# timsainb/noisereduce

Hardware: AMD Instinct MI355X
Metric: Msamples/s reduce_noise (48 kHz mono, n_fft=1024) (higher is better)
Workload: dtype f32

## Files before the change

noisereduce_amd/csrc/api.hip:

```cpp
#include <hip/hip_runtime.h>
#include <dlfcn.h>

#include <algorithm>
#include <cmath>
#include <cstdarg>
#include <cstdio>
#include <cstring>
#include <map>
#include <mutex>
#include <string>
#include <vector>

#include "../../include/mi355gate_debug.h"
#pragma clang fp contract(on)
#include "kernels.hpp"
#include "fused.hpp"
#include "czt.hpp"
#include "mixed.hpp"
#include "onepass.hpp"
#include "rowgate.hpp"
#include "rowbwd.hpp"
#include "fast512.hpp"
#include "onepass512.hpp"
#include "fast256.hpp"
// ... 2147 lines not shown
  P.inv_ktot = 1.0f / (float)h->ktot;
#if OP_WHO
  if (!g_who_dev) HIPCHK(h, hipMalloc((void**)&g_who_dev, 4096 * 16));
  HIPCHK(h, hipMemsetAsync(g_who_dev, 0, 4096 * 16, st));
  P.who = g_who_dev;
#endif
#if OP_TRACE
  {
    static unsigned* tr = nullptr;
    static size_t tr_slots = 0;
    const size_t slots = (size_t)ub * ntt * 4;
    if (!tr || tr_slots < slots) {
      HIPCHK(h, hipMalloc((void**)&tr, slots * 64));
      tr_slots = slots;
      static unsigned** trp = &tr;
      static size_t* trn = &tr_slots;
      static bool reg = false;
      if (!reg) {
        reg = true;
        atexit([] {
          std::vector<unsigned> hst(*trn * 16);
          if (hipMemcpy(hst.data(), *trp, hst.size() * 4, hipMemcpyDeviceToHost) != hipSuccess) return;
          double sum[14] = {0}, w = 0, mx = 0;
          for (size_t i = 0; i < *trn; ++i) {
            if (hst[i * 16 + 15] != 1u) continue;
            w += 1;
            double tot = 0;
            for (int k = 0; k < 14; ++k) { sum[k] += hst[i * 16 + k]; tot += hst[i * 16 + k]; }
            mx = std::max(mx, tot);
          }
          fprintf(stderr, "[OP_TRACE] completed waves %.0f; average shader cycles per wave and phase:", w);
          double tot = 0;
          for (int k = 0; k < 14; ++k) { fprintf(stderr, " %d:%.0f", k, sum[k] / (w > 0 ? w : 1)); tot += sum[k] / (w > 0 ? w : 1); }
          fprintf(stderr, "  sum %.0f  longest wave %.0f\n", tot, mx);
        });
      }
    }
    HIPCHK(h, hipMemsetAsync(tr, 0, slots * 64, st));
    P.trace = tr;
    g_trace_dev = tr; g_trace_tiles = (size_t)ub * ntt; g_trace_ntt = (int)ntt;
  }
#endif
  {
    ProfScope ps(h, SG_STAGE_ONEPASS, st);
    const size_t lds = (size_t)(fast::FN + WAVES * fast::WAVE_CX_H) * sizeof(fast::cf) + (1024 + T2_FLOATS) * sizeof(float) +
                       256 * 8 + 514 * 8 + 32 + (prop ? 528 : 0);
    auto go = [&](auto kern) -> hipError_t {
      hipError_t e = set_lds(reinterpret_cast<const void*>(kern), lds);
      if (e != hipSuccess) return e;
      hipLaunchKernelGGL(kern, dim3(persist ? pgrid : (unsigned)(ub * ntt)), dim3(WAVES * 64), lds, st, P);
      return hipGetLastError();
    };
    if (persist && prop) HIPCHK(h, go(fast::k_gate_onepass<WAVES, true, false, false, true>));
    else if (persist) HIPCHK(h, go(fast::k_gate_onepass<WAVES, false, false, false, true>));
    else if (h->lose_now & 3u) HIPCHK(h, go(fast::k_gate_onepass<WAVES, false, true>));
    else if (prop) HIPCHK(h, go(fast::k_gate_onepass<WAVES, true>));
    else HIPCHK(h, go(fast::k_gate_onepass<WAVES, false>));
  }
  if (lazy) {
    ProfScope ps(h, SG_STAGE_STFT_MAX, st);
    const int wpr = (g.F + 63) / 64;
    HIPCHK(h, launch_bits_any<0>(h, vx, g, ub, tc,
                             (unsigned long long*)h->pmax.p, (unsigned long long*)h->bits.p, wpr, st));
    if ((rc = handoff_next_epoch(h, st))) return rc;
    P.epoch = h->epoch;
    P.ticket = (unsigned*)h->xticket.p + 8;
    P.ticket_base = 0;
    const size_t lds = (size_t)(fast::FN + WAVES * fast::WAVE_CX_H) * sizeof(fast::cf) + (1024 + T2_FLOATS) * sizeof(float) +
                       256 * 8 + 514 * 8 + 32 + (prop ? 528 : 0);
    auto redo = [&](auto kern) -> hipError_t {
      hipError_t e = set_lds(reinterpret_cast<const void*>(kern), lds);
      if (e != hipSuccess) return e;
      hipLaunchKernelGGL(kern, dim3((unsigned)(ub * ntt)), dim3(WAVES * 64), lds, st, P);
      return hipGetLastError();
    };
    if (prop) HIPCHK(h, redo(fast::k_gate_onepass<WAVES, true, false, true>));
    else HIPCHK(h, redo(fast::k_gate_onepass<WAVES, false, false, true>));
    HIPCHK(h, hipGetLastError());
  }
  h->dbg_xbits = true;
  h->dbg_trows = 16; h->dbg_tstep = 16; h->dbg_twords = fast::OP_TILE_WORDS; h->dbg_txw = fast::OP_XW;
  h->dbg_tf0 = A.h_begin - 3;
  h->dbg_ntt = (int)ntt;
  h->dbg_db = std::max<int64_t>(0, A.h_begin - 3 - NF);
  h->dbg_de = std::min<int64_t>(g.T, A.h_begin - 3 + NF * (n_tiles + 1));
  return SG_OK;
}

template <int WAVES, bool KMASK>
static hipError_t launch_apply_fast64(fast::Apply64Args& A, int64_t nh, int64_t ub, hipStream_t st) {
  constexpr int NH = 4 * WAVES - 3;
  const size_t lds = (size_t)(fast::FN + WAVES * 4 * fast::FSLOTS_D + 17) * sizeof(fast::cd);
// ... 1328 lines not shown
```

noisereduce_amd/csrc/onepass.hpp:

```cpp
#pragma once
#include "fastpath.hpp"

namespace sg {
namespace fast {

constexpr int OP_XW = 9;
constexpr int OP_TILE_WORDS = 16 * OP_XW * 2;
constexpr int OP_MAX_NT = 16;
constexpr int OP_KP = 528;
constexpr int OP_TAB_WIN = 0, OP_TAB_WSQ = 4096, OP_TAB_INVN = 8192, OP_TAB_TW512 = 9216, OP_TAB_TW1024 = 13312,
              OP_TAB_WIN64 = 17408, OP_TAB_TW64 = 25600, OP_TAB_MCONST = 33792, OP_TAB_EXP8 = 35328, OP_TAB_BYTES = 37376;

#ifndef OP_LATE_ARGS
#define OP_LATE_ARGS 1
#endif
#ifndef OP_TRACE
#define OP_TRACE 0
#endif
#ifndef OP_ARGCHECK
#define OP_ARGCHECK 0
#endif
#ifndef OP_TILECOUNT
#define OP_TILECOUNT 0
#endif
#ifndef OP_NO_LOOPTOP_WAIT
#define OP_NO_LOOPTOP_WAIT 0
#endif
#ifndef OP_BACKOFF
#define OP_BACKOFF 0
#endif
#if OP_BACKOFF
#define OP_POLL_SLEEP(spin) do { if ((spin) >= 8) __builtin_amdgcn_s_sleep(127); else __builtin_amdgcn_s_sleep(1); } while (0)
#else
#define OP_POLL_SLEEP(spin) __builtin_amdgcn_s_sleep(1)
#endif
#ifndef OP_WHO
#define OP_WHO 0
#endif
#ifndef OP_GLOBAL_DRAW
#define OP_GLOBAL_DRAW 0
#endif
#if OP_GLOBAL_DRAW
#define OP_DRAW_TICKET(p64) __hip_atomic_fetch_add((__attribute__((address_space(1))) unsigned*)(p64), 1u, __ATOMIC_RELAXED, __HIP_MEMORY_SCOPE_AGENT)
#else
#define OP_DRAW_TICKET(p64) atomicAdd((unsigned*)(uintptr_t)(p64), 1u)
#endif
#ifndef OP_DRAW_TOP
#define OP_DRAW_TOP 0
#endif
#ifndef OP_RESTAGE
#define OP_RESTAGE 0
#endif
#ifndef OP_MAX_ITERS
#define OP_MAX_ITERS 0
#endif
#ifndef OP_LATE_START_US
#define OP_LATE_START_US 0
#endif
#ifndef OP_EXP_STALL_NS
#define OP_EXP_STALL_NS 0
#endif
#ifndef OP_INPLACE
#define OP_INPLACE 0
#endif
struct OnePassArgs {
  ApplyArgs A;
  const void* x_exact;
  int64_t stride_exact;
// ... 30 lines not shown
#if OP_LATE_ARGS
  const __attribute__((address_space(4))) char* kp4 = (const __attribute__((address_space(4))) char*)__builtin_amdgcn_kernarg_segment_ptr();
  asm volatile("" : "+s"(kp4));
#endif
  const int64_t s0 = t * OP_XARG(int32_t, A.g.H) - OP_XARG(int32_t, A.g.padL);
  const int64_t v_cs = OP_XARG(int64_t, A.view.cs), v_pad = OP_XARG(int64_t, A.view.pad), v_Lp = OP_XARG(int64_t, A.view.Lp),
                v_lo = OP_XARG(int64_t, A.view.lo), v_hi = OP_XARG(int64_t, A.view.hi), x_stride = OP_XARG(int64_t, stride_exact);
  const void* const x_exact = (const void*)(uintptr_t)OP_XARG(unsigned long long, x_exact);
  const int x_dtype = OP_XARG(int, dtype_exact);
  const char* const tab = (const char*)(uintptr_t)OP_XARG(unsigned long long, tab);
  const int64_t e = chunk * v_cs - v_pad + s0;
  int a, b;
  exact1024_terms(s0, e, v_Lp, v_lo, v_hi, a, b);
  return exact1024_power(x_exact, x_dtype, row * x_stride + e, a, b, reinterpret_cast<const double*>(tab + OP_TAB_WIN64),
                         reinterpret_cast<const cx<double>*>(tab + OP_TAB_TW64), f, lane);
}

__device__ __forceinline__ unsigned op_nan_bits() {
  unsigned v = 0x7fc00000u;
  asm volatile("" : "+v"(v));
  return v;
}

#ifndef OP_ABLATE
#define OP_ABLATE 0
#endif
#ifndef OP_TRACE
#define OP_TRACE 0
#endif
#if OP_TRACE
#define OP_STAMP(i)                                                                                   \
  do {                                                                                                \
    const long long t_now_ = clock64();                                                               \
    if (lane == 0 && t_slot_) t_slot_[i] = (unsigned)(t_now_ - t_prev_);                              \
    t_prev_ = t_now_;                                                                                 \
  } while (0)
#else
#define OP_STAMP(i) do { } while (0)
#endif

#ifndef OP_LATE_P
#define OP_LATE_P 1
#endif
#ifndef OP_OCC
#define OP_OCC 3
#endif
#define OP_DONE { if (PERSIST) continue; return; }
#ifndef OP_DEFER_SEAM
#define OP_DEFER_SEAM 1
#endif
constexpr unsigned OP_SEAM_NONE = 0xffffffffu;
template <int WAVES, bool PROP, bool LOSE = false, bool REDO = false, bool PERSIST = false>
__global__ __launch_bounds__(WAVES * 64, OP_OCC) void k_gate_onepass(OnePassArgs Pk) {
  static_assert(WAVES == 4, "tile = 16 frames");
  static_assert(!PERSIST || (!LOSE && !REDO), "the persistent loop is the lazy first launch only");
  extern __shared__ __attribute__((aligned(16))) char smem[];
  cf* tw512 = reinterpret_cast<cf*>(smem);
  cf* regions = tw512 + FN;
  float* swin = reinterpret_cast<float*>(regions + WAVES * WAVE_CX_H);
  float* s_t2 = swin + 1024;
  unsigned long long* s_exp = reinterpret_cast<unsigned long long*>(s_t2 + T2_FLOATS);
  double* s_t2d = reinterpret_cast<double*>(s_exp + 256);
  unsigned* s_misc = reinterpret_cast<unsigned*>(s_t2d + 514);
  unsigned char* s_ef = reinterpret_cast<unsigned char*>(s_misc + 8);
  constexpr int NF = 4 * WAVES;
  constexpr int SPAN = (NF - 1) * 256 + 1024, XPITCH = 288;
  static_assert((SPAN / 256) * XPITCH <= WAVES * WAVE_CX_H * 2, "span must fit the exchange slices");
  constexpr int NQ = SPAN / 256;
  static_assert(SPAN % 256 == 0 && WAVES * 64 == 256, "one sample per thread and row");
  constexpr int SCAN_REG = 5;

  if (REDO && Pk.alim[1] != Pk.tc.need_tag) return;
#if OP_LATE_START_US
  if (PERSIST && (blockIdx.x % 5u) == 1u) {
    const unsigned long long t0_ = wall_clock64();
    while ((long long)(wall_clock64() - t0_) < (long long)OP_LATE_START_US * 100 * (1 + (blockIdx.x % 7u))) __builtin_amdgcn_s_sleep(8);
  }
#endif
  double t2pre[3];
  unsigned alim_v = 0u;
  {
    const int tid = threadIdx.x, lane = tid & 63;
    static_assert(FN == 2 * WAVES * 64 && WAVES * 64 == 256, "one pass of the prologue loads per thread");
    const cf tw_a = reinterpret_cast<const cf*>(Pk.tab + OP_TAB_TW512)[(tid >> 4) * (tid & 15)];
    const cf tw_b = reinterpret_cast<const cf*>(Pk.tab + OP_TAB_TW512)[((tid + 256) >> 4) * (tid & 15)];
    const float4 w4 = reinterpret_cast<const float4*>(Pk.tab + OP_TAB_WIN)[tid];
    const unsigned long long e8 = reinterpret_cast<const unsigned long long*>(Pk.tab + OP_TAB_EXP8)[tid];
    t2pre[0] = Pk.tc.T2[perm_inv(tid)];
    t2pre[1] = Pk.tc.T2[perm_inv(tid + 256)];
    t2pre[2] = Pk.tc.T2[perm_inv(512)];
    if (!REDO && Pk.alim != nullptr) {
      int z = 2 + min(lane & 15, OP_ALIM_BLOCKS - 1);
      asm volatile("" : "+v"(z));
      alim_v = Pk.alim[z];
    }
    if (tid == 0) {
      s_misc[PERSIST ? 4 : 0] = Pk.ticket_base == 0xffffffffu ? blockIdx.x : atomicAdd(Pk.ticket, 1u) - Pk.ticket_base;
      s_misc[1] = 0u;
      if (PERSIST) s_misc[0] = OP_SEAM_NONE;
    }
    tw512[tid] = tw_a;
    tw512[tid + 256] = tw_b;
    reinterpret_cast<float4*>(swin)[tid] = w4;
    s_exp[tid] = e8;
    if constexpr (PROP) {
      for (int f = tid; f <= 512; f += WAVES * 64) {
        const int lo = max(-Pk.nf, -f), hi = min(Pk.nf, 512 - f);
        int sum = 0;
        for (int a = lo; a <= hi; ++a) sum += Pk.nf + 1 - (a < 0 ? -a : a);
        s_ef[f] = (unsigned char)sum;
      }
    }
    if constexpr (PERSIST) {
#pragma unroll
      for (int k = 0; k < 3; ++k) {
        const int i = tid + k * WAVES * 64;
        if (i > 512) break;
        s_t2[t2_pos(i)] = t2_to_f32(t2pre[k], 4.0);
        s_t2d[i] = t2pre[k];
      }
      for (int off = 1; off < 16; off <<= 1) alim_v = min(alim_v, (unsigned)__shfl_xor((int)alim_v, off));
      if (tid == 0) s_misc[2] = alim_v;
#if OP_TILECOUNT == 2
      if (tid == 0) { s_misc[3] = Pk.total_tiles; s_misc[6] = (unsigned)(uintptr_t)Pk.err; s_misc[7] = (unsigned)((uintptr_t)Pk.err >> 32); }
#endif
    }
  }
// ... 65 lines not shown
                      (rowq * OP_QARG(int64_t, A.om.stride) + gi00 - OP_QARG(int64_t, A.om.g0)));
    src = (const unsigned long long*)uni((const unsigned long long*)(uintptr_t)OP_QARG(unsigned long long, part2) +
                                         ((size_t)uq * ntl + jq - 1) * 3 * 256);
  };
  auto seam_off = [](int wv, int s4_) -> int { return wv * 256 + s4_; };
  auto seam_finish = [&](unsigned pend, int wv, int s4_, unsigned long long g0_, unsigned long long g1_, unsigned long long g2_,
                        unsigned long long g3_, float* dst, float4 ld, float4 nrm) {
    op_v4u ga = {(unsigned)g0_, (unsigned)(g0_ >> 32), (unsigned)g1_, (unsigned)(g1_ >> 32)};
    op_v4u gb = {(unsigned)g2_, (unsigned)(g2_ >> 32), (unsigned)g3_, (unsigned)(g3_ >> 32)};
    typedef const __attribute__((address_space(4))) char* kq_t;
    kq_t kq = (kq_t)__builtin_amdgcn_kernarg_segment_ptr();
    asm volatile("" : "+s"(kq));
    const unsigned e = OP_QARG(unsigned, epoch);
    if (!(ga[1] == e && ga[3] == e && gb[1] == e && gb[3] == e)) {
      const unsigned long long* src;
      float* d2_;
      seam_where(pend, src, d2_);
      src += seam_off(wv, s4_);
      for (int spin = 0;; ++spin) {
        asm volatile("global_load_dwordx4 %0, %2, off sc1\n\tglobal_load_dwordx4 %1, %2, off offset:16 sc1\n\ts_waitcnt vmcnt(0)"
                     : "=&v"(ga), "=&v"(gb) : "v"(src) : "memory");
        if (ga[1] == e && ga[3] == e && gb[1] == e && gb[3] == e) break;
        if (spin >= OP_SPIN_MAX) {
          atomicOr_system((unsigned*)(uintptr_t)OP_QARG(unsigned long long, err), 2u);
          ga[0] = ga[2] = gb[0] = gb[2] = op_nan_bits();
          break;
        }
        OP_POLL_SLEEP(spin);
      }
    }
    const float psn = __uint_as_float((pend >> 31) * 0x7fc00000u);
    float4 a;
    a.x = __uint_as_float(ga[0]) + ld.x;
    a.y = __uint_as_float(ga[2]) + ld.y;
    a.z = __uint_as_float(gb[0]) + ld.z;
    a.w = __uint_as_float(gb[2]) + ld.w;
    a.x = (a.x + psn) * nrm.x; a.y = (a.y + psn) * nrm.y; a.z = (a.z + psn) * nrm.z; a.w = (a.w + psn) * nrm.w;
    *reinterpret_cast<float4*>(dst + seam_off(wv, s4_)) = a;
  };
  auto seam_close = [&](unsigned pend, int tid_) {
    const int wv = tid_ >> 6, s4_ = (tid_ & 63) * 4;
    if (pend == OP_SEAM_NONE || wv >= 3) return;
    typedef const __attribute__((address_space(4))) char* kq_t;
    kq_t kq = (kq_t)__builtin_amdgcn_kernarg_segment_ptr();
    asm volatile("" : "+s"(kq));
    const float4 nrm = *reinterpret_cast<const float4*>(
        &reinterpret_cast<const float*>((const char*)(uintptr_t)OP_QARG(unsigned long long, tab) + OP_TAB_INVN)[s4_]);
    const unsigned long long* src;
    float* dst;
    seam_where(pend, src, dst);
    const float4 ld = *reinterpret_cast<const float4*>(dst + seam_off(wv, s4_));
    seam_finish(pend, wv, s4_, 0ull, 0ull, 0ull, 0ull, dst, ld, nrm);
  };

#if OP_EXP_STALL_NS
  const unsigned long long op_exp_t0_ = wall_clock64();
#endif
  for (unsigned iter = 0; iter == 0u || PERSIST; ++iter) {
  const OnePassArgs& P = (PERSIST || OP_LATE_P) ? *late_args<OnePassArgs>() : Pk;
  int tid = threadIdx.x;
#if OP_ARGCHECK
#if OP_ARGCHECK == 2
  if (PERSIST && threadIdx.x == 1) {
    const unsigned* a_ = reinterpret_cast<const unsigned*>(&P);
    const unsigned* b_ = reinterpret_cast<const unsigned*>(&Pk);
    bool same_ = true;
    for (unsigned w_ = 0; w_ < sizeof(OnePassArgs) / 4; ++w_) same_ = same_ && a_[w_] == b_[w_];
    if (!same_) atomicOr_system(Pk.err, 0x80u);
  }
#else
  if (PERSIST && threadIdx.x == 0 && (P.total_tiles != Pk.total_tiles || P.epoch != Pk.epoch || P.xbits != Pk.xbits || P.A.view.x != Pk.A.view.x))
    atomicOr_system(Pk.err, 0x80u);
#endif
#endif
// ... 29 lines not shown
    atomicOr_system(e_, 0x40u);
    atomicMax_system(e_ + 6, P.total_tiles);
    atomicMax_system(e_ + 7, iter);
  }
  if (PERSIST && ticket >= s_misc[3]) return;
#endif
#if OP_WHO
  if (PERSIST && threadIdx.x == 0 && ticket < 4096u) P.who[ticket * 4 + 2] = (blockIdx.x + 1u) | (iter << 16);
#endif
  if (PERSIST && ticket >= P.total_tiles) {
    if constexpr (DEFER) seam_close((unsigned)__builtin_amdgcn_readfirstlane((int)s_misc[0]), tid);
    return;
  }
#if OP_TILECOUNT == 1
  if (PERSIST && threadIdx.x == 0) { atomicAdd_system(P.err + 4, 1u); atomicAdd_system(P.err + 5, ticket); }
#endif
#if OP_RESTAGE
  if (PERSIST && iter != 0u) {
    const int t_ = threadIdx.x;
    tw512[t_] = reinterpret_cast<const cf*>(P.tab + OP_TAB_TW512)[(t_ >> 4) * (t_ & 15)];
    tw512[t_ + 256] = reinterpret_cast<const cf*>(P.tab + OP_TAB_TW512)[((t_ + 256) >> 4) * (t_ & 15)];
    reinterpret_cast<float4*>(swin)[t_] = reinterpret_cast<const float4*>(P.tab + OP_TAB_WIN)[t_];
    s_exp[t_] = reinterpret_cast<const unsigned long long*>(P.tab + OP_TAB_EXP8)[t_];
#pragma unroll
    for (int k = 0; k < 3; ++k) {
      const int i = t_ + k * WAVES * 64;
      if (i > 512) break;
      const double v_ = P.tc.T2[perm_inv(i)];
      s_t2[t2_pos(i)] = t2_to_f32(v_, 4.0);
      s_t2d[i] = v_;
    }
  }
#endif
  if (PERSIST && tid == 0) {
    s_misc[1] = 0u;
#if OP_TK_LATE
    s_misc[tk_slot ^ 1u] = 0xffffffffu;
#endif
  }
#if OP_TRACE
  t_slot_ = P.trace + ((size_t)ticket * 4 + wave) * 16;
  if (lane == 0) t_slot_[14] = (blockIdx.x + 1u) | (iter << 16);
#endif
  OP_STAMP(0);
  const int64_t u = ticket / (unsigned)ntt;
  const int jt = (int)(ticket % (unsigned)ntt) - 1;
// ... 100 lines not shown
    const float2* wl = reinterpret_cast<const float2*>(swin + 2 * c);
    if (blk_vec) {
#pragma unroll
      for (int r = 0; r < 32; ++r) {
        const float2 x2 = *reinterpret_cast<const float2*>(xs + (r >> 3) * XPITCH + 32 * (r & 7));
        const float2 w2 = wl[16 * r];
        v[r] = {x2.x * w2.x, x2.y * w2.y};
      }
    } else {
#pragma unroll
      for (int r = 0; r < 32; ++r) {
        float2 x2 = *reinterpret_cast<const float2*>(xs + (r >> 3) * XPITCH + 32 * (r & 7));
        if (!fvalid) x2 = make_float2(0.f, 0.f);
        const float2 w2 = wl[16 * r];
        v[r] = {x2.x * w2.x, x2.y * w2.y};
      }
    }
  }
  __syncthreads();
  OP_STAMP(2);
  {
#pragma unroll
    for (int r = 0; r < 32; ++r) nrm2 += v[r].x * v[r].x + v[r].y * v[r].y;
    nrm2 += __shfl_xor(nrm2, 1);
    nrm2 += __shfl_xor(nrm2, 2);
    nrm2 += __shfl_xor(nrm2, 4);
    nrm2 += __shfl_xor(nrm2, 8);
  }
  {
    int z0 = 0;
    asm volatile("" : "+v"(z0));
    fft512_fwd_half(v, fb, tw512 + z0, c);
  }
  OP_STAMP(3);

#if OP_INPLACE
  const bool l0 = c == 0;
  cf wlo = reinterpret_cast<const cf*>(P.tab + OP_TAB_TW1024)[c];
  asm volatile("" : "+v"(wlo.x), "+v"(wlo.y));
  cf whi = wlo;
  {
    const cf w16 = reinterpret_cast<const cf*>(P.tab + OP_TAB_TW1024)[16];
    if (l0) whi = {-w16.y, w16.x};
  }
  rg_lane0_to_entries(v, l0);
  {
    const cf r0 = v[0], r31 = v[31];
    cf xa, xb;
    split_pair(r0, r31, wlo, xa, xb);
    v[0] = {l0 ? r0.x : xa.x, l0 ? r0.y : xa.y};
// ... 104 lines not shown
        const double Pe = op_exact_power(P, row, chunk, tq + gs, f, lane);
        const bool pass = Pe > s_t2d[q < 32 ? cs * 32 + q : 512];
        if (lane == src) {
          if (q < 32) {
            pred = (pred & ~(1u << q)) | ((pass ? 1u : 0u) << q);
            amb &= ~(1u << q);
          } else {
            pred512 = pass;
            amb512 = false;
          }
        }
      }
      wave_lds_sync();
#pragma unroll
      for (int i = 0; i < 16; ++i) {
        OP_PB(i).x = park[(2 * i) * 64];
        OP_PB(i).y = park[(2 * i + 1) * 64];
      }
      wave_lds_sync();
    }
    if (l0)
      pred = (pred & 0xffu) | ((pred & 0x00ffff00u) << 8) | ((pred >> 15) & 0xfe00u) | ((pred >> 23) & 0x100u);
    unsigned tr = pred;
    auto tstep = [&](int sft, unsigned msk, unsigned long long up) {
      const unsigned y = (unsigned)__shfl_xor((int)tr, sft);
      const unsigned ysh = sel_s(up, y >> sft, y << sft);
      const unsigned mk = sel_s(up, msk, ~msk);
      tr = (tr & ~mk) | (ysh & mk);
    };
    tstep(8, 0x00ff00ffu, 0xff00ff00ff00ff00ull);
    tstep(4, 0x0f0f0f0fu, 0xf0f0f0f0f0f0f0f0ull);
    tstep(2, 0x33333333u, 0xccccccccccccccccull);
    tstep(1, 0x55555555u, 0xaaaaaaaaaaaaaaaaull);
    const unsigned long long b8 = __ballot(pred512);
    {
      const int sh = 16 * g;
      const int srcl = (lane & 48) | ((2 * c) & 15);
      const unsigned wa = (unsigned)__shfl((int)tr, srcl), wb2 = (unsigned)__shfl((int)tr, srcl + 1);
      const unsigned f0 = wa & 0xffffu, f1 = wa >> 16, f2 = wb2 & 0xffffu, f3 = wb2 >> 16;
      const unsigned r1 = (((__brev(f1) >> 16) << 1) | (f1 & 1u)) & 0xffffu;
      const unsigned r3 = (((__brev(f3) >> 16) << 1) | (f3 & 1u)) & 0xffffu;
      myword = (unsigned long long)(f0 | (r1 << 16)) | ((unsigned long long)(f2 | (r3 << 16)) << 32);
      if (c == 8) myword = (b8 >> sh) & 1ull;
    }
  }

  OP_STAMP(5);
#if OP_LATE_ARGS
  typedef const __attribute__((address_space(4))) char* op_kpm_t;
  op_kpm_t kpm = (op_kpm_t)__builtin_amdgcn_kernarg_segment_ptr();
  asm volatile("" : "+s"(kpm));
#define OP_MARG(type, member) (*(const __attribute__((address_space(4))) type*)(kpm + __builtin_offsetof(OnePassArgs, member)))
  const unsigned m_ticket = (unsigned)__builtin_amdgcn_readfirstlane((int)s_misc[tk_slot]);
  const unsigned m_ntt = (unsigned)(OP_MARG(int, A.n_tiles) + 2);
  const int64_t m_u = m_ticket / m_ntt;
  const int m_jt = (int)(m_ticket % m_ntt) - 1;
// ... 9 lines not shown
  const char* const m_tab = (const char*)(uintptr_t)OP_MARG(unsigned long long, tab);
  const float m_kscale = OP_MARG(float, A.kscale);
  const int m_nt = OP_MARG(int, nt);
  [[maybe_unused]] const float m_inv_ktot = OP_MARG(float, inv_ktot), m_prop = OP_MARG(float, prop);
  unsigned long long* xb_mine = m_xbits + ((size_t)m_u * m_ntt + (m_jt + 1)) * OP_TILE_WORDS;
  if (c < OP_XW) {
    const op_v4u gr = {(unsigned)myword, m_epoch, (unsigned)(myword >> 32), m_epoch};
    op_st16_sc1(&xb_mine[((4 * wave + g) * OP_XW + c) * 2], gr);
  }
  [[maybe_unused]] unsigned pend_halo = OP_SEAM_NONE;
  if constexpr (DEFER) {
    if (halo_tile) pend_halo = (unsigned)__builtin_amdgcn_readfirstlane((int)s_misc[0]);
  }
  __syncthreads();
  if (halo_tile) {
    if constexpr (DEFER) {
      seam_close(pend_halo, tid);
      if (tid == 0) s_misc[0] = OP_SEAM_NONE;
    }
    if constexpr (PERSIST) {
#if OP_MAX_ITERS == 1 || OP_DRAW_TOP
      if (tid == 0) s_misc[tk_slot ^ 1u] = 0xffffffffu;
#else
      if (tid == 0) s_misc[tk_slot ^ 1u] = OP_DRAW_TICKET(OP_MARG(unsigned long long, ticket)) - OP_MARG(unsigned, ticket_base);
#endif
      pf = false;
#pragma unroll
      for (int k = 0; k < NQ; ++k) q[k] = 0.f;
#pragma unroll
      for (int k = 0; k < SCAN_REG; ++k) sc[k] = 0.f;
    }
    OP_DONE;
  }
  OP_STAMP(6);

  constexpr int WP = OP_XW + 2;
  constexpr int WPB = WP * 8;
  constexpr int SLICE_B = WAVE_CX_H * 8;
  char* rbytes = reinterpret_cast<char*>(regions);
  unsigned long long* wb = reinterpret_cast<unsigned long long*>(rbytes + 4 * OP_KP * 2);
  static_assert(4 * OP_KP * 2 + 48 * WPB <= SLICE_B, "bit rows must fit behind wave 0's K rows");
  const unsigned char* wbb = reinterpret_cast<const unsigned char*>(wb);
  if (c < OP_XW) wb[(m_nt + 4 * wave + g) * WP + 1 + c] = myword;
  for (int r = tid; r < 48; r += WAVES * 64) {
    wb[r * WP] = 0ull;
    wb[r * WP + WP - 1] = 0ull;
  }
  const int q4 = lane >> 4, j16 = lane & 15;
  const long Bf = (long)reinterpret_cast<const unsigned long long*>(m_tab + OP_TAB_MCONST)[lane], At1 = (long)reinterpret_cast<const unsigned long long*>(m_tab + OP_TAB_MCONST)[64 + lane], At2 = (long)reinterpret_cast<const unsigned long long*>(m_tab + OP_TAB_MCONST)[128 + lane];
  const bool three = 2 * m_nt > 16;
  const int m1 = j16, m2 = 16 + j16;
  const int r1 = m1 < 2 * m_nt ? (m1 < m_nt ? m1 : 16 + m1) : 0;
  const int r2 = m2 < 2 * m_nt ? (m2 < m_nt ? m2 : 16 + m2) : 0;
  __syncthreads();
  typedef int op_v4i __attribute__((ext_vector_type(4)));
  const op_v4i zero4 = {0, 0, 0, 0};
  unsigned hown[9];
  {
    const unsigned char* rp = wbb + (m_nt + j16) * WPB + 7 + q4;
#pragma unroll
    for (int nb = 0; nb < 9; ++nb) {
      const int b = wave + 4 * nb;
      hown[nb] = 0u;
      if (b < 33) {
        const long a = (long)s_exp[rp[2 * b]];
        const op_v4i h = __builtin_amdgcn_mfma_i32_16x16x32_i8(a, Bf, zero4, 0, 0, 0);
        hown[nb] = (unsigned)h[0] | ((unsigned)h[1] << 8) | ((unsigned)h[2] << 16) | ((unsigned)h[3] << 24);
      }
    }
  }
  OP_STAMP(7);
  for (int i = tid; i < 2 * m_nt * OP_XW; i += WAVES * 64) {
    const int side = i >= m_nt * OP_XW;
    const int rem = i - side * m_nt * OP_XW;
    const int rr = rem / OP_XW, w = rem - rr * OP_XW;
    const unsigned long long* src = side ? xb_mine + OP_TILE_WORDS + (rr * OP_XW + w) * 2
                                         : xb_mine - OP_TILE_WORDS + ((NF - m_nt + rr) * OP_XW + w) * 2;
    op_v4u gr = op_ld16_sc1(src);
    for (int spin = 0; !(OP_ABLATE & 2) && (LOSE || gr[1] != m_epoch || gr[3] != m_epoch); ++spin) {
      if (LOSE || spin >= OP_SPIN_MAX) {
        atomicOr_system(m_err, 1u);
#if OP_WHO
        if (atomicAdd_system(m_err + 14, 1u) == 0u) { m_err[8] = m_ticket; m_err[9] = (unsigned)i; m_err[10] = gr[1]; m_err[11] = m_epoch; }
#endif
        s_misc[1] = 1u;
        break;
      }
      OP_POLL_SLEEP(spin);
      gr = op_ld16_sc1(src);
    }
    wb[(side ? m_nt + NF + rr : rr) * WP + 1 + w] = (unsigned long long)gr[0] | ((unsigned long long)gr[2] << 32);
  }
  __syncthreads();
  OP_STAMP(8);
  [[maybe_unused]] unsigned nx_raw = 0u;
  if constexpr (PERSIST) {
#if OP_MAX_ITERS == 1 || OP_DRAW_TOP
    if (tid == 0) nx_raw = 0xffffffffu + OP_MARG(unsigned, ticket_base);
#else
    if (tid == 0) nx_raw = OP_DRAW_TICKET(OP_MARG(unsigned long long, ticket));
#endif
  }
  {
    const unsigned char* rp1 = wbb + r1 * WPB + 7 + q4;
    const unsigned char* rp2 = wbb + r2 * WPB + 7 + q4;
#pragma unroll
    for (int nb = 0; nb < 9; ++nb) {
      const int b = wave + 4 * nb;
      if (b < 33) {
        const long a1 = (long)s_exp[rp1[2 * b]];
        const op_v4i h1 = __builtin_amdgcn_mfma_i32_16x16x32_i8(a1, Bf, zero4, 0, 0, 0);
        const unsigned p1 = (unsigned)h1[0] | ((unsigned)h1[1] << 8) | ((unsigned)h1[2] << 16) | ((unsigned)h1[3] << 24);
        const long bt1 = (long)(((unsigned long long)p1 << 32) | (unsigned long long)hown[nb]);
        op_v4i d = __builtin_amdgcn_mfma_i32_16x16x32_i8(At1, bt1, zero4, 0, 0, 0);
        if (three) {
          const long a2 = (long)s_exp[rp2[2 * b]];
          const op_v4i h2 = __builtin_amdgcn_mfma_i32_16x16x32_i8(a2, Bf, zero4, 0, 0, 0);
          const unsigned p2 = (unsigned)h2[0] | ((unsigned)h2[1] << 8) | ((unsigned)h2[2] << 16) | ((unsigned)h2[3] << 24);
          d = __builtin_amdgcn_mfma_i32_16x16x32_i8(At2, (long)(unsigned long long)p2, d, 0, 0, 0);
        }
        unsigned short* kd = reinterpret_cast<unsigned short*>(rbytes + q4 * (SLICE_B + 64)) + 16 * b + j16;
        kd[0] = (unsigned short)d[0];
        kd[OP_KP] = (unsigned short)d[1];
// ... 92 lines not shown
    for (int i = 9; i < 16; ++i) v[i] = sel(pb[16 - i], pa[i]);
#pragma unroll
    for (int i = 16; i < 24; ++i) v[i] = sel(pa[i - 8], pb[31 - i]);
#pragma unroll
    for (int i = 24; i < 31; ++i) v[i] = sel(pb[39 - i], pb[31 - i]);
    v[31] = sel(pb[8], pb[0]);
  }
#endif
  wave_lds_sync();
  OP_STAMP(10);
#if OP_TK_LATE
  if constexpr (PERSIST) {
    if (tid == 0) *(volatile unsigned*)&s_misc[tk_slot ^ 1u] = nx_raw - OP_MARG(unsigned, ticket_base);
  }
#endif

  {
    int zi = 0, ci = c;
    asm volatile("" : "+v"(zi), "+v"(ci));
    fft512_inv_half(v, fb + zi, tw512 + zi, ci);
  }
  OP_STAMP(11);
  float4 n4;
  auto load_n4 = [&]() { n4 = *reinterpret_cast<const float4*>(&reinterpret_cast<const float*>(m_tab + OP_TAB_INVN)[(tid & 63) * 4]); };
  if constexpr (PERSIST) load_n4();
  auto prefetch_next = [&]() {
    const OnePassArgs& Pn = *late_args<OnePassArgs>();
#if OP_TK_LATE
    unsigned nx_v;
    while ((nx_v = *(volatile unsigned*)&s_misc[tk_slot ^ 1u]) == 0xffffffffu) __builtin_amdgcn_s_sleep(1);
    const unsigned nx = (unsigned)__builtin_amdgcn_readfirstlane((int)nx_v);
#else
    const unsigned nx = (unsigned)__builtin_amdgcn_readfirstlane((int)s_misc[tk_slot ^ 1u]);
#endif
    pf = true;
    const bool n_live = nx < Pn.total_tiles;
    const unsigned n_ntt = (unsigned)(Pn.A.n_tiles + 2);
    const unsigned n_tk = n_live ? nx : 0u;
    const unsigned n_u = n_tk / n_ntt;
    const int n_jt = (int)(n_tk % n_ntt) - 1;
    const unsigned n_gu = (unsigned)(Pn.A.view.unit0 + n_u), n_nch = (unsigned)Pn.A.view.n_chunks;
    const TileSrc N = tile_src(Pn, (int64_t)(n_gu / n_nch), Pn.A.view.c0 + n_gu % n_nch, n_jt, true);
    if (n_live && N.blk_vec) {
#pragma unroll
      for (int k = 0; k < NQ; ++k) q[k] = N.sp[tid + k * 256];
    } else {
#pragma unroll
      for (int k = 0; k < NQ; ++k) q[k] = 0.f;
    }
    if (n_live && N.sc_base != nullptr) {
#pragma unroll
      for (int k = 0; k < SCAN_REG; ++k) sc[k] = N.sc_base[min(tid + k * WAVES * 64, N.sc_n1)];
    } else {
#pragma unroll
      for (int k = 0; k < SCAN_REG; ++k) sc[k] = 0.f;
    }
  };
#ifndef OP_PF_AT
#define OP_PF_AT 2
#endif
#ifndef OP_TK_LATE
#define OP_TK_LATE 0
#endif
#ifndef OP_SEAM_AT
#define OP_SEAM_AT 4
#endif
  [[maybe_unused]] unsigned sm_pend = OP_SEAM_NONE;
  [[maybe_unused]] unsigned long long sm_g0 = 0ull, sm_g1 = 0ull, sm_g2 = 0ull, sm_g3 = 0ull;
  [[maybe_unused]] float* sm_dst = nullptr;
  [[maybe_unused]] float4 sm_lead = make_float4(0.f, 0.f, 0.f, 0.f);
  auto seam_issue = [&]() {
    sm_pend = (unsigned)__builtin_amdgcn_readfirstlane((int)s_misc[0]);
    if (sm_pend != OP_SEAM_NONE && wave < 3) {
      const unsigned long long* sm_src;
      seam_where(sm_pend, sm_src, sm_dst);
      sm_src += seam_off(wave, (tid & 63) * 4);
      sm_g0 = __hip_atomic_load((const __attribute__((address_space(1))) unsigned long long*)(sm_src), __ATOMIC_RELAXED, __HIP_MEMORY_SCOPE_AGENT);
      sm_g1 = __hip_atomic_load((const __attribute__((address_space(1))) unsigned long long*)(sm_src + 1), __ATOMIC_RELAXED, __HIP_MEMORY_SCOPE_AGENT);
      sm_g2 = __hip_atomic_load((const __attribute__((address_space(1))) unsigned long long*)(sm_src + 2), __ATOMIC_RELAXED, __HIP_MEMORY_SCOPE_AGENT);
      sm_g3 = __hip_atomic_load((const __attribute__((address_space(1))) unsigned long long*)(sm_src + 3), __ATOMIC_RELAXED, __HIP_MEMORY_SCOPE_AGENT);
      typedef float op_v4f __attribute__((ext_vector_type(4)));
      const op_v4f l4 = *(const __attribute__((address_space(1))) op_v4f*)(sm_dst + seam_off(wave, (tid & 63) * 4));
      sm_lead = make_float4(l4[0], l4[1], l4[2], l4[3]);
    }
  };
  if constexpr (PERSIST && OP_PF_AT == 0) prefetch_next();
  float* acc = reinterpret_cast<float*>(regions + wave * WAVE_CX_H);
  {
    const float2* wsrc2 = reinterpret_cast<const float2*>(swin + 2 * c);
#pragma unroll
    for (int j = 0; j < 4; ++j) {
#pragma unroll
      for (int rr = 0; rr < 8; ++rr) {
        const int r = 8 * j + rr;
        float2* dst = reinterpret_cast<float2*>(acc + (g + j) * HPITCH + 2 * c + 32 * rr);
        const float2 ws = wsrc2[16 * r];
        float2 nw = {v[r].x * ws.x, v[r].y * ws.y};
        if (j != 0) {
          const float2 old = *dst;
          nw.x = sel_s(OLA_KEEP, nw.x + old.x, nw.x);
          nw.y = sel_s(OLA_KEEP, nw.y + old.y, nw.y);
        }
        *dst = nw;
      }
      wave_lds_sync();
      if constexpr (PERSIST) { if (j + 1 == OP_PF_AT) prefetch_next(); }
// ... 42 lines not shown
  const int64_t e_u = u, e_row = row, e_chunk = chunk, e_tf = tf_tile;
  const int e_jt = jt;
  [[maybe_unused]] const unsigned e_ticket = ticket;
#endif
  const float* fr = reinterpret_cast<const float*>(regions);
  const int s4 = (tid & 63) * 4;
  unsigned poison_u = __builtin_amdgcn_readfirstlane((int)s_misc[1]) != 0 ? 0x7fc00000u : 0u;
  asm volatile("" : "+s"(poison_u));
  const float poison = __uint_as_float(poison_u);
  {
    const int64_t pb0 = e_tf * 256 - e_padL;
    const int64_t gi00 = e_chunk * e_gstep + (pb0 - e_p0);
    float* dbase = (float*)e_out + (e_row * e_ostride + gi00 - e_g0);
    float* dst0 = dbase + s4;
    const bool tile_fast = e_odtype == 0 && e_normalize && e_tf >= 3 && e_tf + NF + 2 < e_T &&
                           e_tf >= e_hbegin && e_tf + NF + 2 < e_hend && pb0 >= e_p0 &&
                           pb0 + NF * 256 <= e_p1 && pb0 + NF * 256 <= e_Lout && gi00 >= e_glo &&
                           gi00 + NF * 256 <= e_ghi && (reinterpret_cast<uintptr_t>(dbase) & 15) == 0 && WAVES == 4;
    if (tile_fast) {
      constexpr int R = WAVE_CX_H * 2;
      auto ld4 = [&](int off) { return *reinterpret_cast<const float4*>(&fr[off + s4]); };
      auto fin = [&](float4 a, int jj) {
        a.x = (a.x + poison) * n4.x; a.y = (a.y + poison) * n4.y; a.z = (a.z + poison) * n4.z; a.w = (a.w + poison) * n4.w;
        *reinterpret_cast<float4*>(dst0 + jj * 256) = a;
      };
      if (wave == 3) {
#pragma unroll
        for (int it = 0; it < 4; ++it) fin(ld4(it * R + 3 * HPITCH), 3 + 4 * it);
        OP_STAMP(13);
        if constexpr (PERSIST && OP_PF_AT == 5) prefetch_next();
        OP_DONE;
      }
      {
        const float4 a4 = ld4((WAVES - 1) * R + (wave + 4) * HPITCH);
        unsigned long long* dst = e_part2 + (((size_t)e_u * e_ntiles + e_jt) * 3 + wave) * 256 + s4;
        const op_v4u ga = {__float_as_uint(a4.x + poison), e_epoch, __float_as_uint(a4.y + poison), e_epoch};
        const op_v4u gb = {__float_as_uint(a4.z + poison), e_epoch, __float_as_uint(a4.w + poison), e_epoch};
        op_st16_sc1(dst, ga);
        op_st16_sc1(dst + 2, gb);
      }
#pragma unroll
      for (int it = 1; it < 4; ++it) {
        float4 a4 = ld4((it - 1) * R + (wave + 4) * HPITCH);
        const float4 f4 = ld4(it * R + wave * HPITCH);
        a4.x += f4.x; a4.y += f4.y; a4.z += f4.z; a4.w += f4.w;
        fin(a4, wave + 4 * it);
      }
      if constexpr (DEFER) {
        if (sm_pend != OP_SEAM_NONE) seam_finish(sm_pend, wave, s4, sm_g0, sm_g1, sm_g2, sm_g3, sm_dst, sm_lead, n4);
        *reinterpret_cast<float4*>(dst0 + wave * 256) = ld4(wave * HPITCH);
        if (tid == 0) s_misc[0] = e_ticket | (s_misc[1] != 0u ? 0x80000000u : 0u);
      } else {
        float4 a4 = ld4(wave * HPITCH);
        const unsigned long long* src = e_part2 + (((size_t)e_u * e_ntiles + e_jt - 1) * 3 + wave) * 256 + s4;
        op_v4u ga, gb;
        for (int spin = 0;; ++spin) {
          asm volatile("global_load_dwordx4 %0, %2, off sc1\n\tglobal_load_dwordx4 %1, %2, off offset:16 sc1\n\ts_waitcnt vmcnt(0)"
                       : "=&v"(ga), "=&v"(gb) : "v"(src) : "memory");
          const unsigned e = e_epoch;
          if ((OP_ABLATE & 16) || (!LOSE && ga[1] == e && ga[3] == e && gb[1] == e && gb[3] == e)) break;
          if (LOSE || spin >= OP_SPIN_MAX) {
            atomicOr_system(e_err, 2u);
#if OP_WHO
            if (atomicAdd_system(e_err + 15, 1u) == 0u) { e_err[12] = e_ticket; e_err[13] = ga[1]; }
#endif
            ga[0] = ga[2] = gb[0] = gb[2] = op_nan_bits();
            break;
          }
          OP_POLL_SLEEP(spin);
        }
        a4.x = __uint_as_float(ga[0]) + a4.x;
        a4.y = __uint_as_float(ga[2]) + a4.y;
        a4.z = __uint_as_float(gb[0]) + a4.z;
        a4.w = __uint_as_float(gb[2]) + a4.w;
        fin(a4, wave);
      }
      OP_STAMP(13);
      if constexpr (PERSIST && OP_PF_AT == 5) prefetch_next();
      OP_DONE;
    }
  }
  if constexpr (DEFER) {
    if (sm_pend != OP_SEAM_NONE && wave < 3) seam_finish(sm_pend, wave, s4, sm_g0, sm_g1, sm_g2, sm_g3, sm_dst, sm_lead, n4);
    if (tid == 0) s_misc[0] = OP_SEAM_NONE;
  }
// ... 17 lines not shown
      if (wh < WAVES) {
        const float4 f4 = *reinterpret_cast<const float4*>(&fr[wh * WAVE_CX_H * 2 + lh * HPITCH + s4]);
        a4.x += f4.x; a4.y += f4.y; a4.z += f4.z; a4.w += f4.w;
      }
    }
    if (jj >= NF) {
      const int k = jj - NF;
      unsigned long long* dst = e_part2 + (((size_t)e_u * e_ntiles + e_jt) * 3 + k) * 256 + s4;
      const op_v4u ga = {__float_as_uint(a4.x + poison), e_epoch, __float_as_uint(a4.y + poison), e_epoch};
      const op_v4u gb = {__float_as_uint(a4.z + poison), e_epoch, __float_as_uint(a4.w + poison), e_epoch};
      op_st16_sc1(dst, ga);
      op_st16_sc1(dst + 2, gb);
      continue;
    }
    if (jj < 3) {
      const unsigned long long* src = e_part2 + (((size_t)e_u * e_ntiles + e_jt - 1) * 3 + jj) * 256 + s4;
      op_v4u ga, gb;
      for (int spin = 0;; ++spin) {
        asm volatile("global_load_dwordx4 %0, %2, off sc1\n\tglobal_load_dwordx4 %1, %2, off offset:16 sc1\n\ts_waitcnt vmcnt(0)"
                     : "=&v"(ga), "=&v"(gb) : "v"(src) : "memory");
        const unsigned e = e_epoch;
        if ((OP_ABLATE & 16) || (!LOSE && ga[1] == e && ga[3] == e && gb[1] == e && gb[3] == e)) break;
        if (LOSE || spin >= OP_SPIN_MAX) {
          atomicOr_system(e_err, 2u);
          ga[0] = ga[2] = gb[0] = gb[2] = op_nan_bits();
          break;
        }
        OP_POLL_SLEEP(spin);
      }
      a4.x = __uint_as_float(ga[0]) + a4.x;
      a4.y = __uint_as_float(ga[2]) + a4.y;
      a4.z = __uint_as_float(gb[0]) + a4.z;
      a4.w = __uint_as_float(gb[2]) + a4.w;
    }
    a4.x += poison; a4.y += poison; a4.z += poison; a4.w += poison;
    if (!e_normalize) {
    } else if (all_valid) {
      a4.x *= n4.x; a4.y *= n4.y; a4.z *= n4.z; a4.w *= n4.w;
    } else {
      float4 nrm = make_float4(0.f, 0.f, 0.f, 0.f);
#pragma unroll
      for (int q = 0; q < 4; ++q) {
        const int64_t ti = h - q;
        if (ti >= 0 && ti < e_T) {
          const float4 w4 = *reinterpret_cast<const float4*>(&reinterpret_cast<const float*>(e_tab + OP_TAB_WSQ)[256 * q + s4]);
          nrm.x += w4.x; nrm.y += w4.y; nrm.z += w4.z; nrm.w += w4.w;
        }
// ... 35 lines not shown
```

Baseline: 104,800.

## Trim wait-count stalls in onepass kernel via global address space and LDS constants

Several small changes aim to reduce s_waitcnt stalls in the persistent onepass gate kernel. Stores and loads to output use explicit global address-space pointers rather than flat pointers. The ticket atomic is issued as a global agent-scope atomic, and the error atomics become global-scoped. The MCONST table is staged into LDS once per block rather than read from global each tile. Half-wave shuffles are replaced with ds_swizzle, and the prefetch branches are replaced with unconditional loads from a stand-in pointer. Per-wave trace reporting is also added. The cost is extra LDS per block and loads that always run, even when only a stand-in is needed.

```diff
diff --git a/noisereduce_amd/csrc/api.hip b/noisereduce_amd/csrc/api.hip
--- a/noisereduce_amd/csrc/api.hip
+++ b/noisereduce_amd/csrc/api.hip
@@ -2193,12 +2193,19 @@
           std::vector<unsigned> hst(*trn * 16);
           if (hipMemcpy(hst.data(), *trp, hst.size() * 4, hipMemcpyDeviceToHost) != hipSuccess) return;
           double sum[14] = {0}, w = 0, mx = 0;
+          double wsum[4][14] = {{0}}, ww[4] = {0};
           for (size_t i = 0; i < *trn; ++i) {
             if (hst[i * 16 + 15] != 1u) continue;
             w += 1;
+            ww[i & 3] += 1;
             double tot = 0;
-            for (int k = 0; k < 14; ++k) { sum[k] += hst[i * 16 + k]; tot += hst[i * 16 + k]; }
+            for (int k = 0; k < 14; ++k) { sum[k] += hst[i * 16 + k]; wsum[i & 3][k] += hst[i * 16 + k]; tot += hst[i * 16 + k]; }
             mx = std::max(mx, tot);
+          }
+          for (int wv = 0; wv < 4; ++wv) {
+            fprintf(stderr, "[OP_TRACE] wave %d (%.0f completed):", wv, ww[wv]);
+            for (int k = 0; k < 14; ++k) fprintf(stderr, " %d:%.0f", k, wsum[wv][k] / (ww[wv] > 0 ? ww[wv] : 1));
+            fprintf(stderr, "\n");
           }
           fprintf(stderr, "[OP_TRACE] completed waves %.0f; average shader cycles per wave and phase:", w);
           double tot = 0;
@@ -2215,7 +2222,7 @@
   {
     ProfScope ps(h, SG_STAGE_ONEPASS, st);
     const size_t lds = (size_t)(fast::FN + WAVES * fast::WAVE_CX_H) * sizeof(fast::cf) + (1024 + T2_FLOATS) * sizeof(float) +
-                       256 * 8 + 514 * 8 + 32 + (prop ? 528 : 0);
+                       256 * 8 + 514 * 8 + 192 * 8 + 32 + (prop ? 528 : 0);
     auto go = [&](auto kern) -> hipError_t {
       hipError_t e = set_lds(reinterpret_cast<const void*>(kern), lds);
       if (e != hipSuccess) return e;
@@ -2238,7 +2245,7 @@
     P.ticket = (unsigned*)h->xticket.p + 8;
     P.ticket_base = 0;
     const size_t lds = (size_t)(fast::FN + WAVES * fast::WAVE_CX_H) * sizeof(fast::cf) + (1024 + T2_FLOATS) * sizeof(float) +
-                       256 * 8 + 514 * 8 + 32 + (prop ? 528 : 0);
+                       256 * 8 + 514 * 8 + 192 * 8 + 32 + (prop ? 528 : 0);
     auto redo = [&](auto kern) -> hipError_t {
       hipError_t e = set_lds(reinterpret_cast<const void*>(kern), lds);
       if (e != hipSuccess) return e;
diff --git a/noisereduce_amd/csrc/onepass.hpp b/noisereduce_amd/csrc/onepass.hpp
--- a/noisereduce_amd/csrc/onepass.hpp
+++ b/noisereduce_amd/csrc/onepass.hpp
@@ -36,14 +36,6 @@
 #endif
 #ifndef OP_WHO
 #define OP_WHO 0
-#endif
-#ifndef OP_GLOBAL_DRAW
-#define OP_GLOBAL_DRAW 0
-#endif
-#if OP_GLOBAL_DRAW
-#define OP_DRAW_TICKET(p64) __hip_atomic_fetch_add((__attribute__((address_space(1))) unsigned*)(p64), 1u, __ATOMIC_RELAXED, __HIP_MEMORY_SCOPE_AGENT)
-#else
-#define OP_DRAW_TICKET(p64) atomicAdd((unsigned*)(uintptr_t)(p64), 1u)
 #endif
 #ifndef OP_DRAW_TOP
 #define OP_DRAW_TOP 0
@@ -120,6 +112,44 @@
   return v;
 }
 
+#ifndef OP_WAIT_SITES
+#define OP_WAIT_SITES 7
+#endif
+typedef float op_v4f __attribute__((ext_vector_type(4)));
+#if OP_WAIT_SITES & 2
+#define OP_G4 __attribute__((address_space(1)))
+#else
+#define OP_G4
+#endif
+__device__ __forceinline__ float4 op_ldg4(const float* p) {
+  const op_v4f v = *(const OP_G4 op_v4f*)p;
+  return make_float4(v[0], v[1], v[2], v[3]);
+}
+__device__ __forceinline__ void op_stg4(float* p, float4 a) {
+  const op_v4f v = {a.x, a.y, a.z, a.w};
+  *(OP_G4 op_v4f*)p = v;
+}
+__device__ __forceinline__ unsigned op_draw_ticket_late(unsigned long long p64) {
+#if OP_WAIT_SITES & 1
+  asm volatile("" : "+v"(p64));
+  return __hip_atomic_fetch_add((__attribute__((address_space(1))) unsigned*)p64, 1u, __ATOMIC_RELAXED, __HIP_MEMORY_SCOPE_AGENT);
+#else
+  return atomicAdd((unsigned*)(uintptr_t)p64, 1u);
+#endif
+}
+
+__device__ __forceinline__ void op_err_or(unsigned* p, unsigned bits) {
+  __HIP_ATOMIC_BACKWARD_COMPAT_MEMORY {
+    __hip_atomic_fetch_or((__attribute__((address_space(1))) unsigned*)p, bits, __ATOMIC_RELAXED, __HIP_MEMORY_SCOPE_SYSTEM);
+  }
+}
+
+template <int M>
+__device__ __forceinline__ int op_xor_lanes(int v) {
+  static_assert(M > 0 && M < 32, "within a half-wave");
+  return __builtin_amdgcn_ds_swizzle(v, (M << 10) | 0x1f);
+}
+
 #ifndef OP_ABLATE
 #define OP_ABLATE 0
 #endif
@@ -159,7 +189,8 @@
   float* s_t2 = swin + 1024;
   unsigned long long* s_exp = reinterpret_cast<unsigned long long*>(s_t2 + T2_FLOATS);
   double* s_t2d = reinterpret_cast<double*>(s_exp + 256);
-  unsigned* s_misc = reinterpret_cast<unsigned*>(s_t2d + 514);
+  unsigned long long* s_mc = reinterpret_cast<unsigned long long*>(s_t2d + 514);
+  unsigned* s_misc = reinterpret_cast<unsigned*>(s_mc + 192);
   unsigned char* s_ef = reinterpret_cast<unsigned char*>(s_misc + 8);
   constexpr int NF = 4 * WAVES;
   constexpr int SPAN = (NF - 1) * 256 + 1024, XPITCH = 288;
@@ -184,6 +215,7 @@
     const cf tw_b = reinterpret_cast<const cf*>(Pk.tab + OP_TAB_TW512)[((tid + 256) >> 4) * (tid & 15)];
     const float4 w4 = reinterpret_cast<const float4*>(Pk.tab + OP_TAB_WIN)[tid];
     const unsigned long long e8 = reinterpret_cast<const unsigned long long*>(Pk.tab + OP_TAB_EXP8)[tid];
+    const unsigned long long mc8 = reinterpret_cast<const unsigned long long*>(Pk.tab + OP_TAB_MCONST)[min(tid, 191)];
     t2pre[0] = Pk.tc.T2[perm_inv(tid)];
     t2pre[1] = Pk.tc.T2[perm_inv(tid + 256)];
     t2pre[2] = Pk.tc.T2[perm_inv(512)];
@@ -201,6 +233,7 @@
     tw512[tid + 256] = tw_b;
     reinterpret_cast<float4*>(swin)[tid] = w4;
     s_exp[tid] = e8;
+    if (tid < 192) s_mc[tid] = mc8;
     if constexpr (PROP) {
       for (int f = tid; f <= 512; f += WAVES * 64) {
         const int lo = max(-Pk.nf, -f), hi = min(Pk.nf, 512 - f);
@@ -312,7 +345,7 @@
                      : "=&v"(ga), "=&v"(gb) : "v"(src) : "memory");
         if (ga[1] == e && ga[3] == e && gb[1] == e && gb[3] == e) break;
         if (spin >= OP_SPIN_MAX) {
-          atomicOr_system((unsigned*)(uintptr_t)OP_QARG(unsigned long long, err), 2u);
+          op_err_or((unsigned*)(uintptr_t)OP_QARG(unsigned long long, err), 2u);
           ga[0] = ga[2] = gb[0] = gb[2] = op_nan_bits();
           break;
         }
@@ -326,7 +359,7 @@
     a.z = __uint_as_float(gb[0]) + ld.z;
     a.w = __uint_as_float(gb[2]) + ld.w;
     a.x = (a.x + psn) * nrm.x; a.y = (a.y + psn) * nrm.y; a.z = (a.z + psn) * nrm.z; a.w = (a.w + psn) * nrm.w;
-    *reinterpret_cast<float4*>(dst + seam_off(wv, s4_)) = a;
+    op_stg4(dst + seam_off(wv, s4_), a);
   };
   auto seam_close = [&](unsigned pend, int tid_) {
     const int wv = tid_ >> 6, s4_ = (tid_ & 63) * 4;
@@ -334,12 +367,11 @@
     typedef const __attribute__((address_space(4))) char* kq_t;
     kq_t kq = (kq_t)__builtin_amdgcn_kernarg_segment_ptr();
     asm volatile("" : "+s"(kq));
-    const float4 nrm = *reinterpret_cast<const float4*>(
-        &reinterpret_cast<const float*>((const char*)(uintptr_t)OP_QARG(unsigned long long, tab) + OP_TAB_INVN)[s4_]);
+    const float4 nrm = op_ldg4(&reinterpret_cast<const float*>((const char*)(uintptr_t)OP_QARG(unsigned long long, tab) + OP_TAB_INVN)[s4_]);
     const unsigned long long* src;
     float* dst;
     seam_where(pend, src, dst);
-    const float4 ld = *reinterpret_cast<const float4*>(dst + seam_off(wv, s4_));
+    const float4 ld = op_ldg4(dst + seam_off(wv, s4_));
     seam_finish(pend, wv, s4_, 0ull, 0ull, 0ull, 0ull, dst, ld, nrm);
   };
 
@@ -415,6 +447,7 @@
     tw512[t_ + 256] = reinterpret_cast<const cf*>(P.tab + OP_TAB_TW512)[((t_ + 256) >> 4) * (t_ & 15)];
     reinterpret_cast<float4*>(swin)[t_] = reinterpret_cast<const float4*>(P.tab + OP_TAB_WIN)[t_];
     s_exp[t_] = reinterpret_cast<const unsigned long long*>(P.tab + OP_TAB_EXP8)[t_];
+    if (t_ < 192) s_mc[t_] = reinterpret_cast<const unsigned long long*>(P.tab + OP_TAB_MCONST)[t_];
 #pragma unroll
     for (int k = 0; k < 3; ++k) {
       const int i = t_ + k * WAVES * 64;
@@ -561,10 +594,10 @@
   {
 #pragma unroll
     for (int r = 0; r < 32; ++r) nrm2 += v[r].x * v[r].x + v[r].y * v[r].y;
-    nrm2 += __shfl_xor(nrm2, 1);
-    nrm2 += __shfl_xor(nrm2, 2);
-    nrm2 += __shfl_xor(nrm2, 4);
-    nrm2 += __shfl_xor(nrm2, 8);
+    nrm2 += __int_as_float(op_xor_lanes<1>(__float_as_int(nrm2)));
+    nrm2 += __int_as_float(op_xor_lanes<2>(__float_as_int(nrm2)));
+    nrm2 += __int_as_float(op_xor_lanes<4>(__float_as_int(nrm2)));
+    nrm2 += __int_as_float(op_xor_lanes<8>(__float_as_int(nrm2)));
   }
   {
     int z0 = 0;
@@ -715,16 +748,15 @@
     if (l0)
       pred = (pred & 0xffu) | ((pred & 0x00ffff00u) << 8) | ((pred >> 15) & 0xfe00u) | ((pred >> 23) & 0x100u);
     unsigned tr = pred;
-    auto tstep = [&](int sft, unsigned msk, unsigned long long up) {
-      const unsigned y = (unsigned)__shfl_xor((int)tr, sft);
+    auto tstep = [&](unsigned y, int sft, unsigned msk, unsigned long long up) {
       const unsigned ysh = sel_s(up, y >> sft, y << sft);
       const unsigned mk = sel_s(up, msk, ~msk);
       tr = (tr & ~mk) | (ysh & mk);
     };
-    tstep(8, 0x00ff00ffu, 0xff00ff00ff00ff00ull);
-    tstep(4, 0x0f0f0f0fu, 0xf0f0f0f0f0f0f0f0ull);
-    tstep(2, 0x33333333u, 0xccccccccccccccccull);
-    tstep(1, 0x55555555u, 0xaaaaaaaaaaaaaaaaull);
+    tstep((unsigned)op_xor_lanes<8>((int)tr), 8, 0x00ff00ffu, 0xff00ff00ff00ff00ull);
+    tstep((unsigned)op_xor_lanes<4>((int)tr), 4, 0x0f0f0f0fu, 0xf0f0f0f0f0f0f0f0ull);
+    tstep((unsigned)op_xor_lanes<2>((int)tr), 2, 0x33333333u, 0xccccccccccccccccull);
+    tstep((unsigned)op_xor_lanes<1>((int)tr), 1, 0x55555555u, 0xaaaaaaaaaaaaaaaaull);
     const unsigned long long b8 = __ballot(pred512);
     {
       const int sh = 16 * g;
@@ -780,7 +812,7 @@
 #if OP_MAX_ITERS == 1 || OP_DRAW_TOP
       if (tid == 0) s_misc[tk_slot ^ 1u] = 0xffffffffu;
 #else
-      if (tid == 0) s_misc[tk_slot ^ 1u] = OP_DRAW_TICKET(OP_MARG(unsigned long long, ticket)) - OP_MARG(unsigned, ticket_base);
+      if (tid == 0) s_misc[tk_slot ^ 1u] = op_draw_ticket_late(OP_MARG(unsigned long long, ticket)) - OP_MARG(unsigned, ticket_base);
 #endif
       pf = false;
 #pragma unroll
@@ -805,7 +837,12 @@
     wb[r * WP + WP - 1] = 0ull;
   }
   const int q4 = lane >> 4, j16 = lane & 15;
-  const long Bf = (long)reinterpret_cast<const unsigned long long*>(m_tab + OP_TAB_MCONST)[lane], At1 = (long)reinterpret_cast<const unsigned long long*>(m_tab + OP_TAB_MCONST)[64 + lane], At2 = (long)reinterpret_cast<const unsigned long long*>(m_tab + OP_TAB_MCONST)[128 + lane];
+#if OP_WAIT_SITES & 4
+  const long Bf = (long)s_mc[lane], At1 = (long)s_mc[64 + lane], At2 = (long)s_mc[128 + lane];
+#else
+  const unsigned long long* const mc_ = reinterpret_cast<const unsigned long long*>(m_tab + OP_TAB_MCONST);
+  const long Bf = (long)mc_[lane], At1 = (long)mc_[64 + lane], At2 = (long)mc_[128 + lane];
+#endif
   const bool three = 2 * m_nt > 16;
   const int m1 = j16, m2 = 16 + j16;
   const int r1 = m1 < 2 * m_nt ? (m1 < m_nt ? m1 : 16 + m1) : 0;
@@ -837,7 +874,7 @@
     op_v4u gr = op_ld16_sc1(src);
     for (int spin = 0; !(OP_ABLATE & 2) && (LOSE || gr[1] != m_epoch || gr[3] != m_epoch); ++spin) {
       if (LOSE || spin >= OP_SPIN_MAX) {
-        atomicOr_system(m_err, 1u);
+        op_err_or(m_err, 1u);
 #if OP_WHO
         if (atomicAdd_system(m_err + 14, 1u) == 0u) { m_err[8] = m_ticket; m_err[9] = (unsigned)i; m_err[10] = gr[1]; m_err[11] = m_epoch; }
 #endif
@@ -856,7 +893,7 @@
 #if OP_MAX_ITERS == 1 || OP_DRAW_TOP
     if (tid == 0) nx_raw = 0xffffffffu + OP_MARG(unsigned, ticket_base);
 #else
-    if (tid == 0) nx_raw = OP_DRAW_TICKET(OP_MARG(unsigned long long, ticket));
+    if (tid == 0) nx_raw = op_draw_ticket_late(OP_MARG(unsigned long long, ticket));
 #endif
   }
   {
@@ -995,7 +1032,7 @@
   }
   OP_STAMP(11);
   float4 n4;
-  auto load_n4 = [&]() { n4 = *reinterpret_cast<const float4*>(&reinterpret_cast<const float*>(m_tab + OP_TAB_INVN)[(tid & 63) * 4]); };
+  auto load_n4 = [&]() { n4 = op_ldg4(&reinterpret_cast<const float*>(m_tab + OP_TAB_INVN)[(tid & 63) * 4]); };
   if constexpr (PERSIST) load_n4();
   auto prefetch_next = [&]() {
     const OnePassArgs& Pn = *late_args<OnePassArgs>();
@@ -1014,20 +1051,15 @@
     const int n_jt = (int)(n_tk % n_ntt) - 1;
     const unsigned n_gu = (unsigned)(Pn.A.view.unit0 + n_u), n_nch = (unsigned)Pn.A.view.n_chunks;
     const TileSrc N = tile_src(Pn, (int64_t)(n_gu / n_nch), Pn.A.view.c0 + n_gu % n_nch, n_jt, true);
-    if (n_live && N.blk_vec) {
-#pragma unroll
-      for (int k = 0; k < NQ; ++k) q[k] = N.sp[tid + k * 256];
-    } else {
-#pragma unroll
-      for (int k = 0; k < NQ; ++k) q[k] = 0.f;
-    }
-    if (n_live && N.sc_base != nullptr) {
-#pragma unroll
-      for (int k = 0; k < SCAN_REG; ++k) sc[k] = N.sc_base[min(tid + k * WAVES * 64, N.sc_n1)];
-    } else {
-#pragma unroll
-      for (int k = 0; k < SCAN_REG; ++k) sc[k] = 0.f;
-    }
+    static_assert(NQ * 256 * 4 <= OP_TAB_BYTES, "the stand-in loads stay inside the tables");
+    const bool n_vec = n_live && N.blk_vec, n_scan = n_live && N.sc_base != nullptr;
+    const float* const n_sp = n_vec ? N.sp : reinterpret_cast<const float*>(Pn.tab);
+    const float* const n_sc = n_scan ? N.sc_base : n_sp;
+    const int n_sc1 = n_scan ? N.sc_n1 : 0;
+#pragma unroll
+    for (int k = 0; k < NQ; ++k) q[k] = n_sp[tid + k * 256];
+#pragma unroll
+    for (int k = 0; k < SCAN_REG; ++k) sc[k] = n_sc[min(tid + k * WAVES * 64, n_sc1)];
   };
 #ifndef OP_PF_AT
 #define OP_PF_AT 2
@@ -1052,9 +1084,7 @@
       sm_g1 = __hip_atomic_load((const __attribute__((address_space(1))) unsigned long long*)(sm_src + 1), __ATOMIC_RELAXED, __HIP_MEMORY_SCOPE_AGENT);
       sm_g2 = __hip_atomic_load((const __attribute__((address_space(1))) unsigned long long*)(sm_src + 2), __ATOMIC_RELAXED, __HIP_MEMORY_SCOPE_AGENT);
       sm_g3 = __hip_atomic_load((const __attribute__((address_space(1))) unsigned long long*)(sm_src + 3), __ATOMIC_RELAXED, __HIP_MEMORY_SCOPE_AGENT);
-      typedef float op_v4f __attribute__((ext_vector_type(4)));
-      const op_v4f l4 = *(const __attribute__((address_space(1))) op_v4f*)(sm_dst + seam_off(wave, (tid & 63) * 4));
-      sm_lead = make_float4(l4[0], l4[1], l4[2], l4[3]);
+      sm_lead = op_ldg4(sm_dst + seam_off(wave, (tid & 63) * 4));
     }
   };
   if constexpr (PERSIST && OP_PF_AT == 0) prefetch_next();
@@ -1143,7 +1173,7 @@
       auto ld4 = [&](int off) { return *reinterpret_cast<const float4*>(&fr[off + s4]); };
       auto fin = [&](float4 a, int jj) {
         a.x = (a.x + poison) * n4.x; a.y = (a.y + poison) * n4.y; a.z = (a.z + poison) * n4.z; a.w = (a.w + poison) * n4.w;
-        *reinterpret_cast<float4*>(dst0 + jj * 256) = a;
+        op_stg4(dst0 + jj * 256, a);
       };
       if (wave == 3) {
 #pragma unroll
@@ -1169,7 +1199,7 @@
       }
       if constexpr (DEFER) {
         if (sm_pend != OP_SEAM_NONE) seam_finish(sm_pend, wave, s4, sm_g0, sm_g1, sm_g2, sm_g3, sm_dst, sm_lead, n4);
-        *reinterpret_cast<float4*>(dst0 + wave * 256) = ld4(wave * HPITCH);
+        op_stg4(dst0 + wave * 256, ld4(wave * HPITCH));
         if (tid == 0) s_misc[0] = e_ticket | (s_misc[1] != 0u ? 0x80000000u : 0u);
       } else {
         float4 a4 = ld4(wave * HPITCH);
@@ -1181,7 +1211,7 @@
           const unsigned e = e_epoch;
           if ((OP_ABLATE & 16) || (!LOSE && ga[1] == e && ga[3] == e && gb[1] == e && gb[3] == e)) break;
           if (LOSE || spin >= OP_SPIN_MAX) {
-            atomicOr_system(e_err, 2u);
+            op_err_or(e_err, 2u);
 #if OP_WHO
             if (atomicAdd_system(e_err + 15, 1u) == 0u) { e_err[12] = e_ticket; e_err[13] = ga[1]; }
 #endif
@@ -1245,7 +1275,7 @@
         const unsigned e = e_epoch;
         if ((OP_ABLATE & 16) || (!LOSE && ga[1] == e && ga[3] == e && gb[1] == e && gb[3] == e)) break;
         if (LOSE || spin >= OP_SPIN_MAX) {
-          atomicOr_system(e_err, 2u);
+          op_err_or(e_err, 2u);
           ga[0] = ga[2] = gb[0] = gb[2] = op_nan_bits();
           break;
         }
```

Measured after the change: 107,600, median of 6. 1.03x the previous value.
